# songyb111-gachon/binary-hologram-reinforcement-learning

Measured on AMD Instinct MI355X. Metric: env-steps/sec (1024x1024, 24-plane), higher is better.
Workload: dtype f32

## Files before the change

### binary-hologram-reinforcement-learning_amd/csrc/hbx_passes.hip

```cpp
#include <hip/hip_runtime.h>
#include <stdint.h>

#include "hbx_fft.hpp"
#include "hbx_internal.hpp"
#include "hbx_rowcol.hpp"
#include "hbx_walk_planes.hpp"

namespace hbx {

template <int SK>
__device__ __forceinline__ float2 store_round(float2 v) {
  if constexpr (SK == HBX_PRECISION_BF16_STORE) {
    auto r = [](float x) {
      uint32_t u = __float_as_uint(x);
      u += 0x7fffu + ((u >> 16) & 1u);
      return __uint_as_float(u & 0xffff0000u);
    };
    return make_float2(r(v.x), r(v.y));
  } else if constexpr (SK == HBX_PRECISION_F16_STORE) {
    return make_float2((float)(_Float16)v.x, (float)(_Float16)v.y);
  } else {
    return v;
  }
}

template <int SK>
__device__ __forceinline__ float2 store_round_a(float2 v) {
  if constexpr (SK == HBX_PRECISION_F16_STORE) {
    return make_float2(2.0f * (float)(_Float16)(0.5f * v.x), 2.0f * (float)(_Float16)(0.5f * v.y));
  } else {
    return store_round<SK>(v);
  }
}

template <int R>
constexpr int kRowNT = row_nt(R);

template <int R>
constexpr int kPanel = panel_rows(R);

template <int R>
using LayoutA = PanelLine<R, R * R / 2, pan_a(R)>;
template <int R>
using LayoutB = PanelLine<R, R * R, pan_b(R)>;

template <int R>
struct TileB {
  static constexpr int N = R * R, TL = 256 / R;
  __device__ static constexpr int at(int s, int y) {
    return (y >> 4) * 16 * N + (s / TL) * 16 * TL + (y & 15) * TL + s % TL;
  }
};
template <int R>
constexpr bool kTiledB = R == 32 || R == 16;



template <int R>
constexpr int rowfwd_iters() { return R == 32 ? 4 : (R == 16 ? 2 : 1); }

__device__ __forceinline__ JobDesc first_pass_job(const JobDesc* jobs, const int64_t* actions, int32_t* err,
                                                  int j, bool writer, int64_t hw, int P, int CH) {
  if (!actions) return jobs[j];
  const JobDesc jb = job_of_action(actions[j], j, hw, P, CH);
  if (writer && threadIdx.x == 0) {
    const_cast<JobDesc*>(jobs)[j] = jb;
    if (jb.env < 0 && err) atomicOr(err, 1);
  }
  return jb;
}

template <int R, int NT>
constexpr int rowfwd_scratch() {
  static_assert(R * R * (NT / R) <= (NT / R) * R * (R + 1), "tile must fit in the scratch area");
  return (NT / R) * R * (R + 1);
}

template <int R, int NT, int SK>
__device__ __forceinline__ void rowfwd_emit(pk2 (&v)[R], int t, int grp, int lane_base, int y0, float2* lds,
                                            const float2* tw, float2* __restrict__ base) {
  constexpr int N = R * R;
  constexpr int GPB = NT / R;
  constexpr size_t PLA = plane_a_elems(R);
  fft_group<R, false>(v, t, PaddedScratch<R>{lds + grp * R * (R + 1)}, tw);
  lds_barrier();

  float2* tile = lds;
  const float2 zny = from_pk(v[R / 2]);
#pragma unroll
  for (int k2 = 0; k2 < R / 2; ++k2) {
    const float2 z = from_pk(v[k2]);
    const float2 m = mirror_conj<R>(v, k2, t, lane_base);
    float2 fa = make_float2(z.x + m.x, z.y + m.y);
    float2 fb = make_float2(z.y - m.y, m.x - z.x);
    if (k2 == 0 && t == 0) {
      fa = make_float2(z.x + z.x, zny.x + zny.x);
      fb = make_float2(z.y + z.y, zny.y + zny.y);
    }
    const int kx = t + R * k2;
    tile[tile_pos<R, GPB>(kx, grp)] = fa;
    tile[tile_pos<R, GPB>(N / 2 + kx, grp)] = fb;
  }
  lds_barrier();
  constexpr int CHUNKS = N * GPB / 2;
  static_assert(CHUNKS % NT == 0, "chunking");
#pragma unroll
  for (int i = 0; i < CHUNKS / NT; ++i) {
    const int c = threadIdx.x + NT * i;
    const int r2 = (c % (GPB / 2)) * 2;
    const int line = c / (GPB / 2);
    float2 a, b;
    if constexpr (GPB == 16) {
      const int p0 = tile_pos<R, GPB>(line, r2);
      const float4 ab = *reinterpret_cast<const float4*>(tile + (p0 & ~1));
      const bool sw = (p0 & 1) != 0;
      a = sw ? make_float2(ab.z, ab.w) : make_float2(ab.x, ab.y);
      b = sw ? make_float2(ab.x, ab.y) : make_float2(ab.z, ab.w);
    } else {
      a = tile[tile_pos<R, GPB>(line, r2)];
      b = tile[tile_pos<R, GPB>(line, r2 + 1)];
    }
    a = store_round_a<SK>(a);
    b = store_round_a<SK>(b);
    const int pl = line / (N / 2);
    st_stream4(base + (size_t)pl * PLA + LayoutA<R>::at(line - pl * (N / 2), y0 + r2),
               make_float4(a.x, a.y, b.x, b.y));
  }
}

template <int R, int NT, int SK, int RIT = rowfwd_iters<R>()>
__global__ __launch_bounds__(NT, 512 / NT) void k_rowfwd(const JobDesc* jobs,
                                                   const uint32_t* __restrict__ mask,
                                                   float2* __restrict__ ws_a,
                                                   const float2* __restrict__ tw_glob, int P,
                                                   int CH, float va, float vb, int pair_step,
                                                   const int64_t* __restrict__ actions, int32_t* err,
                                                   const uint8_t* __restrict__ phase) {
  constexpr int N = R * R;
  constexpr int GPB = NT / R;
  constexpr int WPR = N / 32;
  __shared__ float2 tw[N];
  __shared__ __attribute__((aligned(16))) float2 lds[rowfwd_scratch<R, NT>()];

  stage_twiddles<N, NT>(tw, tw_glob);

  const int grp = threadIdx.x / R;
  const int t = threadIdx.x % R;
  const int lane_base = (threadIdx.x & 63) - t;
  constexpr int RB = N / GPB;
  constexpr int RBW = RB / RIT;
  const FirstPassBlock wg = first_pass_block<RBW>(RIT == 1 ? xcd_pair<RB>(blockIdx.x) : (int)blockIdx.x,
                                                  pair_step ? 1 : P / 2);
  const int rbw = wg.rbw, j = wg.j;
  const JobDesc jb = first_pass_job(jobs, actions, err, j, wg.writer, (int64_t)N * N, P, CH);
  if (jb.env < 0 || (phase && phase[j])) return;
  const int q = pair_step ? (jb.flip_plane >> 1) : wg.q;
  const int pa = 2 * q, pb = 2 * q + 1;
  const uint32_t* plane_a = mask + ((size_t)jb.env * CH + jb.group * P + pa) * N * WPR;
  uint32_t wa[WPR], wb[WPR];
  auto load_row = [&](int y) {
    const uint32_t* rowa = plane_a + (size_t)y * WPR;
    const uint32_t* rowb = rowa + (size_t)N * WPR;
    if constexpr (WPR % 4 == 0) {
#pragma unroll
      for (int i = 0; i < WPR / 4; ++i) {
        const uint4 a = reinterpret_cast<const uint4*>(rowa)[i];
        const uint4 b = reinterpret_cast<const uint4*>(rowb)[i];
        wa[4 * i] = a.x; wa[4 * i + 1] = a.y; wa[4 * i + 2] = a.z; wa[4 * i + 3] = a.w;
        wb[4 * i] = b.x; wb[4 * i + 1] = b.y; wb[4 * i + 2] = b.z; wb[4 * i + 3] = b.w;
      }
    } else {
#pragma unroll
      for (int i = 0; i < WPR; ++i) { wa[i] = rowa[i]; wb[i] = rowb[i]; }
    }
  };
  load_row(rbw * RIT * GPB + grp);
  __syncthreads();

  float2* base = ws_a + ((size_t)j * P + pa) * plane_a_elems(R);
  int it = 0;
#pragma unroll 1
  do {
    const int y0 = (rbw * RIT + it) * GPB;
    const int y = y0 + grp;
    if (jb.flip_plane >= 0 && jb.flip_pix / N == y) {
      const int col = jb.flip_pix % N;
      const uint32_t bit = 1u << (col & 31);
#pragma unroll
      for (int i = 0; i < WPR; ++i) {
        if (i == (col >> 5)) {
          if (jb.flip_plane == pa) wa[i] ^= bit;
          if (jb.flip_plane == pb) wb[i] ^= bit;
        }
      }
    }
    pk2 v[R];
    with_field_kind(va, vb, [&](auto fk) {
#pragma unroll
      for (int jj = 0; jj < R; ++jj) {
        const int w = (R * jj) >> 5;
        const int sh = ((R * jj) & 31) + t;
        v[jj] = (pk2){bit_value<fk()>(wa[w], sh, va, vb), bit_value<fk()>(wb[w], sh, va, vb)};
      }
    });
    if constexpr (RIT > 1) {
      load_row(it + 1 < RIT ? y + GPB : y);
      if (it > 0) lds_barrier();
    }
    rowfwd_emit<R, NT, SK>(v, t, grp, lane_base, y0, lds, tw, base);
  } while (RIT > 1 && ++it < RIT);
}

constexpr int kRowfwd32Scr = 8 * 32 * (32 + 1);
static_assert((1024 / 2) * 8 * 2 <= kRowfwd32Scr, "one plane's tile must fit in the FFT tiles");

template <int SK>
__device__ __forceinline__ void rowfwd32_emit(pk2 (&v)[32], int t, int k1, int grp, int y0, float* lds,
                                              const float2* tw, float2* __restrict__ base) {
  constexpr int R = 32, NT = 256, N = R * R, GPB = NT / R;
  constexpr size_t PLA = plane_a_elems(R);
  float2* tile = reinterpret_cast<float2*>(lds);
  fft_group_split_mirror<false>(v, t, k1, lds + grp * R * (R + 1), tw);

  float2 fb[R / 2];
  lds_barrier();
  const float2 zny = from_pk(v[R / 2]);
#pragma unroll
  for (int k2 = 0; k2 < R / 2; ++k2) {
    const float2 z = from_pk(v[k2]);
    const float2 m = mirror_conj_paired(v, k2, t);
    float2 fa = make_float2(z.x + m.x, z.y + m.y);
    fb[k2] = make_float2(z.y - m.y, m.x - z.x);
    if (k2 == 0 && t == 0) {
      fa = make_float2(z.x + z.x, zny.x + zny.x);
      fb[k2] = make_float2(z.y + z.y, zny.y + zny.y);
    }
    tile[tile_pos<R, GPB>(k1 + R * k2, grp)] = fa;
  }
  constexpr int CHUNKS = (N / 2) * GPB / 2;
  static_assert(CHUNKS % NT == 0, "chunking");
#pragma unroll
  for (int pl = 0; pl < 2; ++pl) {
    if (pl == 1) {
      lds_barrier();
#pragma unroll
      for (int k2 = 0; k2 < R / 2; ++k2) tile[tile_pos<R, GPB>(k1 + R * k2, grp)] = fb[k2];
    }
    lds_barrier();
#pragma unroll
    for (int i = 0; i < CHUNKS / NT; ++i) {
      const int c = threadIdx.x + NT * i;
      const int r2 = (c % (GPB / 2)) * 2;
      const int line = c / (GPB / 2);
      const float2 a = store_round_a<SK>(tile[tile_pos<R, GPB>(line, r2)]);
      const float2 b = store_round_a<SK>(tile[tile_pos<R, GPB>(line, r2 + 1)]);
      st_stream4(base + (size_t)pl * PLA + LayoutA<R>::at(line, y0 + r2), make_float4(a.x, a.y, b.x, b.y));
    }
  }
}

template <int SK, int RIT = rowfwd_iters<32>()>
__global__ __launch_bounds__(256, 3) void k_rowfwd32(const JobDesc* jobs,
                                                     const uint32_t* __restrict__ mask,
                                                     float2* __restrict__ ws_a,
                                                     const float2* __restrict__ tw_glob, int P, int CH,
                                                     float va, float vb, int pair_step,
                                                     const int64_t* __restrict__ actions, int32_t* err,
                                                     const uint8_t* __restrict__ phase) {
  constexpr int R = 32, NT = 256, N = R * R;
  constexpr int GPB = NT / R;
  constexpr int WPR = N / 32;
  __shared__ float2 tw[N];
  __shared__ __attribute__((aligned(16))) float lds[kRowfwd32Scr];

  stage_twiddles<N, NT>(tw, tw_glob);

  const int grp = threadIdx.x / R;
  const int t = threadIdx.x % R;
  const int k1 = mirror_k1(t);
  constexpr int RB = N / GPB;
  constexpr int RBW = RB / RIT;
  int bid = RIT == 1 ? xcd_pair<RB>(blockIdx.x) : (int)blockIdx.x;
  const int rbw = bid % RBW;
  bid /= RBW;
  const int npair = pair_step ? 1 : P / 2;
  const int j = bid / npair;
  const JobDesc jb = first_pass_job(jobs, actions, err, j, rbw == 0 && bid % npair == 0, (int64_t)N * N, P, CH);
  if (jb.env < 0 || (phase && phase[j])) return;
  const int q = pair_step ? (jb.flip_plane >> 1) : bid % npair;
  const int pa = 2 * q, pb = 2 * q + 1;
  const uint32_t* plane_a = mask + ((size_t)jb.env * CH + jb.group * P + pa) * N * WPR;
  uint32_t wa, wb;
  auto load_row = [&](int y) {
    wa = plane_a[(size_t)y * WPR + t];
    wb = plane_a[(size_t)(N + y) * WPR + t];
  };
  load_row(rbw * RIT * GPB + grp);
  __syncthreads();

  float2* base = ws_a + ((size_t)j * P + pa) * plane_a_elems(R);
  int it = 0;
#pragma unroll 1
  do {
    const int y0 = (rbw * RIT + it) * GPB;
    const int y = y0 + grp;
    uint32_t ta = group_bit_transpose(wa, t);
    uint32_t tb = group_bit_transpose(wb, t);
    if (jb.flip_plane >= 0 && jb.flip_pix / N == y) {
      const int col = jb.flip_pix % N;
      if (t == (col & 31)) {
        if (jb.flip_plane == pa) ta ^= 1u << (col >> 5);
        if (jb.flip_plane == pb) tb ^= 1u << (col >> 5);
      }
    }
    pk2 v[R];
    with_field_kind(va, vb, [&](auto fk) {
#pragma unroll
      for (int jj = 0; jj < R; ++jj)
        v[jj] = (pk2){bit_value<fk()>(ta, jj, va, vb), bit_value<fk()>(tb, jj, va, vb)};
    });
    if constexpr (RIT > 1) {
      load_row(it + 1 < RIT ? y + GPB : y);
      if (it > 0) lds_barrier();
    }
    rowfwd32_emit<SK>(v, t, k1, grp, y0, lds, tw, base);
  } while (RIT > 1 && ++it < RIT);
}

template <int R, int NT>
__global__ __launch_bounds__(NT, 512 / NT) void k_rowfwd_real(const JobDesc* __restrict__ jobs,
                                                        const float* __restrict__ values,
                                                        float2* __restrict__ ws_a,
                                                        const float2* __restrict__ tw_glob, int P, int CH) {
  constexpr int N = R * R;
  constexpr int GPB = NT / R;
  __shared__ float2 tw[N];
  __shared__ __attribute__((aligned(16))) float2 lds[rowfwd_scratch<R, NT>()];

  stage_twiddles<N, NT>(tw, tw_glob);

  const int grp = threadIdx.x / R;
  const int t = threadIdx.x % R;
  const int lane_base = (threadIdx.x & 63) - t;
  constexpr int RB = N / GPB;
  const FirstPassBlock wg = first_pass_block<RB>(xcd_pair<RB>(blockIdx.x), P / 2);
  const int j = wg.j;
  const JobDesc jb = jobs[j];
  if (jb.env < 0) return;
  const int pa = 2 * wg.q;
  const int y0 = wg.rbw * GPB;
  const int y = y0 + grp;
  pk2 v[R];
  real_load_row<R>(v, values + (((size_t)jb.env * CH + jb.group * P + pa) * N + y) * N, (size_t)N * N, t);
  __syncthreads();

  float2* base = ws_a + ((size_t)j * P + pa) * plane_a_elems(R);
  rowfwd_emit<R, NT, HBX_PRECISION_F32>(v, t, grp, lane_base, y0, lds, tw, base);
}

__global__ __launch_bounds__(256, 3) void k_rowfwd32_real(const JobDesc* __restrict__ jobs,
                                                          const float* __restrict__ values,
                                                          float2* __restrict__ ws_a,
                                                          const float2* __restrict__ tw_glob, int P, int CH) {
  constexpr int R = 32, NT = 256, N = R * R;
  constexpr int GPB = NT / R;
  __shared__ float2 tw[N];
  __shared__ __attribute__((aligned(16))) float lds[kRowfwd32Scr];

  stage_twiddles<N, NT>(tw, tw_glob);

  const int grp = threadIdx.x / R;
  const int t = threadIdx.x % R;
  const int k1 = mirror_k1(t);
  constexpr int RB = N / GPB;
  const FirstPassBlock wg = first_pass_block<RB>(xcd_pair<RB>(blockIdx.x), P / 2);
  const int j = wg.j;
  const JobDesc jb = jobs[j];
  if (jb.env < 0) return;
  const int pa = 2 * wg.q;
  const int y0 = wg.rbw * GPB;
  const int y = y0 + grp;
  pk2 v[R];
  real_load_row<R>(v, values + (((size_t)jb.env * CH + jb.group * P + pa) * N + y) * N, (size_t)N * N, t);
  __syncthreads();

  float2* base = ws_a + ((size_t)j * P + pa) * plane_a_elems(R);
  rowfwd32_emit<HBX_PRECISION_F32>(v, t, k1, grp, y0, lds, tw, base);
}

template <int R, int NT, bool WT = false>
__global__ __launch_bounds__(NT, 512 / NT) void k_rowfwd_cplx(const JobDesc* __restrict__ jobs,
                                                        const float2* __restrict__ values,
                                                        float2* __restrict__ ws_a,
                                                        const float2* __restrict__ tw_glob, int P, int CH,
                                                        const float* __restrict__ weight, float scale) {
  constexpr int N = R * R;
  constexpr int GPB = NT / R;
  __shared__ float2 tw[N];
  __shared__ __attribute__((aligned(16))) float2 lds[rowfwd_scratch<R, NT>()];

  stage_twiddles<N, NT>(tw, tw_glob);

  const int grp = threadIdx.x / R;
  const int t = threadIdx.x % R;
  const int lane_base = (threadIdx.x & 63) - t;
  constexpr int RB = N / GPB;
  const FirstPassBlock wg = first_pass_block<RB>(xcd_pair<RB>(blockIdx.x), P / 2);
  const int j = wg.j;
  const JobDesc jb = jobs[j];
  if (jb.env < 0) return;
  const int y0 = wg.rbw * GPB;
  const int y = y0 + grp;
  pk2 v[R];
  const float2* row = values + (((size_t)jb.env * (CH / 2) + jb.group * (P / 2) + wg.q) * N + y) * N;
  if constexpr (WT)
    complex_load_row_weighted<R>(v, row, weight + (((size_t)jb.env * (CH / P) + jb.group) * N + y) * N, scale, t);
  else
    complex_load_row<R>(v, row, t);
  __syncthreads();

  float2* base = ws_a + ((size_t)j * P + 2 * wg.q) * plane_a_elems(R);
  rowfwd_emit<R, NT, HBX_PRECISION_F32>(v, t, grp, lane_base, y0, lds, tw, base);
}

template <bool WT = false>
__global__ __launch_bounds__(256, 3) void k_rowfwd32_cplx(const JobDesc* __restrict__ jobs,
                                                          const float2* __restrict__ values,
                                                          float2* __restrict__ ws_a,
                                                          const float2* __restrict__ tw_glob, int P, int CH,
                                                          const float* __restrict__ weight, float scale) {
  constexpr int R = 32, NT = 256, N = R * R;
  constexpr int GPB = NT / R;
  __shared__ float2 tw[N];
  __shared__ __attribute__((aligned(16))) float lds[kRowfwd32Scr];

  stage_twiddles<N, NT>(tw, tw_glob);

  const int grp = threadIdx.x / R;
  const int t = threadIdx.x % R;
  const int k1 = mirror_k1(t);
  constexpr int RB = N / GPB;
  const FirstPassBlock wg = first_pass_block<RB>(xcd_pair<RB>(blockIdx.x), P / 2);
  const int j = wg.j;
  const JobDesc jb = jobs[j];
  if (jb.env < 0) return;
  const int y0 = wg.rbw * GPB;
  const int y = y0 + grp;
  pk2 v[R];
  const float2* row = values + (((size_t)jb.env * (CH / 2) + jb.group * (P / 2) + wg.q) * N + y) * N;
  if constexpr (WT)
    complex_load_row_weighted<R>(v, row, weight + (((size_t)jb.env * (CH / P) + jb.group) * N + y) * N, scale, t);
  else
    complex_load_row<R>(v, row, t);
  __syncthreads();

  float2* base = ws_a + ((size_t)j * P + 2 * wg.q) * plane_a_elems(R);
  rowfwd32_emit<HBX_PRECISION_F32>(v, t, k1, grp, y0, lds, tw, base);
}

template <int R>
__host__ __device__ constexpr int col2_iters() { return R == 32 ? 4 : (R == 16 ? 2 : 1); }

template <int R, int SK>
__device__ __forceinline__ void col2_stage_write(const float2 (&v)[R], float sy, float2* scratch, int grp, int t) {
  constexpr int PQ = R >= 32 ? 1 : 32 / R;
  float2* reg = col2_region<R>(scratch, grp);
  float2* base[PQ];
#pragma unroll
  for (int q = 0; q < PQ; ++q) base[q] = reg + col2_pos<R>(grp >> 1, t + R * q);
#pragma unroll
  for (int q = 0; q < PQ; ++q) {
#pragma unroll
    for (int k2 = q; k2 < R; k2 += PQ) base[q][R * (k2 - q)] = store_round<SK>(make_float2(v[k2].x, sy * v[k2].y));
  }
}

template <int R, int SK, int ITER = col2_iters<R>()>
__global__ __launch_bounds__(256, 2) void k_col2(const JobDesc* __restrict__ jobs,
                                                 const float2* __restrict__ ws_a,
                                                 float2* __restrict__ ws_b,
                                                 const float2* __restrict__ htab,
                                                 const float2* __restrict__ tw_glob, int P,
                                                 int pair_step, const uint8_t* __restrict__ phase) {
  constexpr int N = R * R;
  constexpr int GPB = 256 / R;
  constexpr int LB = (N / 2) / (GPB * ITER);
  static_assert((N / 2) % (GPB * ITER) == 0, "line blocking");
  __shared__ float2 tw[N];
  constexpr int RS = kTiledB<R> ? col2_region_stride<R>() : R * (R + 1);
  __shared__ float2 scratch[GPB * RS];

  for (int i = threadIdx.x; i < N; i += 256) tw[i] = tw_glob[i];

  const int grp = threadIdx.x / R;
  const int t = threadIdx.x % R;
  const int lane_base = (threadIdx.x & 63) - t;
  int bid = blockIdx.x;
  const int lb = bid % LB;
  bid /= LB;
  const int np = pair_step ? 2 : P;
  const int j = bid / np;
  const JobDesc jb = jobs[j];
  if (jb.env < 0 || (phase && phase[j])) return;
  const int p = pair_step ? (jb.flip_plane & ~1) + bid % 2 : bid % np;
  using PA = LayoutA<R>;
  using PB = LayoutB<R>;
  const __amdgpu_buffer_rsrc_t ra = plane_rsrc(ws_a + ((size_t)j * P + p) * plane_a_elems(R), plane_a_elems(R) * 8);
  const __amdgpu_buffer_rsrc_t rb = plane_rsrc(ws_b + ((size_t)j * P + p) * plane_b_elems(R), plane_b_elems(R) * 8);
  const __amdgpu_buffer_rsrc_t rh = plane_rsrc(htab + (size_t)jb.group * (N / 2 + 1) * N, (N / 2 + 1) * N * 8);
  const PaddedScratch<R> sc{scratch + grp * RS};
  constexpr int KSTEP = LB * GPB;
  const int kx0 = lb * GPB + grp;

  float2 v[R];
  {
    const int vo = PA::voff(t, kx0);
#pragma unroll
    for (int jj = 0; jj < R; ++jj) v[jj] = buf_ld2s(ra, vo, PA::joff(jj));
  }
  lds_barrier();

#pragma unroll 1
  for (int it = 0; it < ITER; ++it) {
    const int kx = kx0 + it * KSTEP;
    const bool dc = (kx == 0);
    const int vh = (kx * N + t) * 8;
    constexpr int HP = kTiledB<R> ? R / 2 + 1 : 0;
    float2 hb[R];
    if constexpr (kTiledB<R>) {
      fft_group_s1<R, false, true>(v, t, tw);
      if (!dc) {
#pragma unroll
        for (int i = 0; i < HP; ++i) hb[i] = buf_ld2(rh, vh, i * R * 8);
      }
      if (it > 0) lds_barrier();
      fft_group_s2<R, false, true>(v, t, sc);
    } else {
      fft_group<R, false, true>(v, t, sc, tw);
    }
    float2 w[R];
    if (!dc) {
      if constexpr (kTiledB<R>) {
        float2* hs = scratch + grp * RS;
        wave_sync();
#pragma unroll
        for (int i = 0; i <= R / 2; ++i) hs[i * R + t] = hb[i];
        wave_sync();
        const float2* hm = hs + (t == 0 ? R : 0) + ((R - t) & (R - 1));
#pragma unroll
        for (int i = R / 2 + 1; i < R; ++i) hb[i] = hm[(R - 1 - i) * R];
        wave_sync();
      } else {
#pragma unroll
        for (int i = 0; i < R; ++i) hb[i] = buf_ld2(rh, vh, i * R * 8);
      }
#pragma unroll
      for (int i = 0; i < R; ++i) {
        w[i] = cmulc(v[i], hb[i]);
        v[i] = cmul(v[i], hb[i]);
      }
    } else {
      const int vn = ((N / 2) * N + t) * 8;
#pragma unroll
      for (int k2 = 0; k2 < R; ++k2) w[k2] = mirror_conj<R>(v, k2, t, lane_base);
#pragma unroll
      for (int k2 = 0; k2 < R; ++k2) {
        const float2 z = v[k2], mm = w[k2];
        v[k2] = cmul(make_float2(0.5f * (z.x + mm.x), 0.5f * (z.y + mm.y)), buf_ld2(rh, vh, k2 * R * 8));
        w[k2] = cmul(make_float2(0.5f * (z.y - mm.y), -0.5f * (z.x - mm.x)), buf_ld2(rh, vn, k2 * R * 8));
      }
    }
    fft_group<R, true, true>(v, t, sc, tw);
    const float sy = dc ? 1.0f : -1.0f;
    if constexpr (kTiledB<R>) {
      const int kxb = kx - grp;
      col2_stage_write<R, SK>(v, 1.0f, scratch, grp, t);
      lds_barrier();
      col2_stage_store<R>(scratch, rb, kxb / GPB);
      if (it + 1 < ITER) {
        const int vo = PA::voff(t, kx + KSTEP);
#pragma unroll
        for (int jj = 0; jj < R; ++jj) v[jj] = buf_ld2s(ra, vo, PA::joff(jj));
      }
      fft_group_s1<R, true, true>(w, t, tw);
      lds_barrier();
      fft_group_s2<R, true, true>(w, t, sc);
      col2_stage_write<R, SK>(w, sy, scratch, grp, t);
      lds_barrier();
      col2_stage_store<R>(scratch, rb, (N / 2 + kxb) / GPB);
    } else {
      {
        const int vo = PB::voff(t, kx);
#pragma unroll
        for (int k2 = 0; k2 < R; ++k2) buf_st2s(store_round<SK>(v[k2]), rb, vo, PB::joff(k2));
      }
      if (it + 1 < ITER) {
        const int vo = PA::voff(t, kx + KSTEP);
#pragma unroll
        for (int jj = 0; jj < R; ++jj) v[jj] = buf_ld2s(ra, vo, PA::joff(jj));
      }
      fft_group<R, true, true>(w, t, sc, tw);
      {
        const int vo = PB::voff(t, dc ? N / 2 : N - kx);
#pragma unroll
        for (int k2 = 0; k2 < R; ++k2)
          buf_st2s(store_round<SK>(make_float2(w[k2].x, sy * w[k2].y)), rb, vo, PB::joff(k2));
      }
    }
  }
}

template <int R, int GPB, bool SC1 = false, bool TPRE = false>
__device__ __forceinline__ void rowinv_epilogue(float (&acc)[R], int P, int G, const JobDesc& jb, int j, int y,
                                                int rb, int grp, int t, const float* __restrict__ target,
                                                size_t tmask, float* __restrict__ inten_out, int inten_by_env,
                                                double* __restrict__ partial, double (&red)[GPB][3],
                                                const int32_t* __restrict__ rc_pending = nullptr,
                                                float* __restrict__ rc_cache = nullptr,
                                                const float* tpre = nullptr) {
  constexpr int N = R * R;
  constexpr int RB = N / GPB;
  const float invp = 1.0f / (float)P;
  const float* trow = target + ((((size_t)jb.env * G + jb.group) * N + y) * N & tmask);
  double sxy = 0.0, sxx = 0.0, syy = 0.0;
#pragma unroll
  for (int k = 0; k < R; ++k) {
    const float I = acc[k] * invp;
    const float T = TPRE ? tpre[k] : trow[t + R * k];
    sxy = fma((double)I, (double)T, sxy);
    sxx = fma((double)I, (double)I, sxx);
    syy = fma((double)T, (double)T, syy);
    acc[k] = I;
  }
  if (inten_out) {
    const size_t slot = inten_by_env ? (size_t)jb.env * G + jb.group : (size_t)j;
    float* orow = inten_out + (slot * N + y) * N;
    if (rc_pending) {
      const int p = rc_pending[jb.env];
      if (p != 0) {
        const int gp = (p > 0 ? p : -p) - 1;
        const size_t grow = (((size_t)jb.env * G + gp) * N + y) * N;
        if (p > 0) {
#pragma unroll
          for (int k = 0; k < R; ++k) rc_cache[grow + t + R * k] = inten_out[grow + t + R * k];
        } else if (gp != jb.group) {
#pragma unroll
          for (int k = 0; k < R; ++k) inten_out[grow + t + R * k] = rc_cache[grow + t + R * k];
        }
      }
    }
    if (inten_by_env) {
#pragma unroll
      for (int k = 0; k < R; ++k) __builtin_nontemporal_store(acc[k], orow + t + R * k);
    } else {
#pragma unroll
      for (int k = 0; k < R; ++k) orow[t + R * k] = acc[k];
    }
  }
#pragma unroll
  for (int off = R / 2; off >= 1; off >>= 1) {
    sxy += __shfl_xor(sxy, off, 64);
    sxx += __shfl_xor(sxx, off, 64);
    syy += __shfl_xor(syy, off, 64);
  }
  if (t == 0) { red[grp][0] = sxy; red[grp][1] = sxx; red[grp][2] = syy; }
  __syncthreads();
  if (threadIdx.x == 0) {
    double a = 0.0, b = 0.0, cc = 0.0;
    for (int g = 0; g < GPB; ++g) { a += red[g][0]; b += red[g][1]; cc += red[g][2]; }
    double* o = partial + ((size_t)j * RB + rb) * 3;
    if constexpr (SC1) {
      const __amdgpu_buffer_rsrc_t ro = walk_planes_rsrc(o, 24);
      __builtin_amdgcn_raw_buffer_store_b64(__builtin_bit_cast(u32x2, a), ro, 0, 0, kSc1Bit);
      __builtin_amdgcn_raw_buffer_store_b64(__builtin_bit_cast(u32x2, b), ro, 8, 0, kSc1Bit);
      __builtin_amdgcn_raw_buffer_store_b64(__builtin_bit_cast(u32x2, cc), ro, 16, 0, kSc1Bit);
    } else {
      o[0] = a; o[1] = b; o[2] = cc;
    }
  }
}

template <int R>
struct RowinvLanes {
  static constexpr int N = R * R, TL = 256 / R;
  static constexpr int JS = 16 * R * 8;
  int lo, hiB, vmid;
  __device__ __forceinline__ RowinvLanes(int y, int t) {
    const int yb = (y >> 4) * 16 * N + (y & 15) * TL;
    const int m = t / TL, u = t % TL;
    lo = (yb + m * 16 * TL + u) * 8;
    hiB = (yb + (u ? (3 * N / (2 * TL) - m - 1) * 16 * TL + TL - u : (3 * N / (2 * TL) - m) * 16 * TL) -
           16 * R * (R - 1)) * 8;
    vmid = t == 0 ? lo + JS * (R / 2) : hiB + JS * (R / 2 - 1);
  }
  __device__ __forceinline__ float2 load(__amdgpu_buffer_rsrc_t rs, int po, int jj) const {
    const int vo = jj < R / 2 ? lo : (jj == R / 2 ? vmid : hiB);
    const int so = po + (jj < R / 2 ? JS * jj : (jj == R / 2 ? 0 : JS * (R - 1 - jj)));
    return buf_ld2s(rs, vo, so);
  }
};

template <int R, bool WALK = false, bool LEAN = false>
__global__ __launch_bounds__(256, 2) void k_rowinv_d(const JobDesc* __restrict__ jobs,
                                                     const float2* __restrict__ ws_b,
                                                     const float* __restrict__ target,
                                                     const float2* __restrict__ tw_glob, int P, int G,
                                                     double* __restrict__ partial, float* __restrict__ inten_out,
                                                     float2* __restrict__ field_out, size_t tmask, int inten_by_env,
                                                     int plane_mode, float* __restrict__ plane_pool,
                                                     const int32_t* __restrict__ plane_slot, int plane_spares,
                                                     int spare_base, const int32_t* __restrict__ rc_pending,
                                                     float* __restrict__ rc_cache, WalkPlanesArgs wk) {
  constexpr int N = R * R, GPB = 256 / R, RB = N / GPB;
  static_assert(!WALK || walk_planes_lds_bytes(RB) <= GPB * R * (R + 1) * 8, "the decision's LDS fits the scratch");
  __shared__ float2 tw[N];
  __shared__ float2 scratch[GPB * R * (R + 1)];
  __shared__ double red[GPB][3];
  for (int i = threadIdx.x; i < N; i += 256) tw[i] = tw_glob[i];

  const int grp = threadIdx.x / R;
  const int t = threadIdx.x % R;
  const int bid = xcd_pair<RB>(blockIdx.x);
  const int rb = bid % RB;
  const int j = bid / RB;
  const JobDesc jb = jobs[j];
  if constexpr (WALK) {
    if (wk.phase && wk.phase[j] == 2) {
      walk_planes_arrive(wk, reinterpret_cast<char*>(scratch));
      return;
    }
  }
  if (jb.env < 0) {
    if (threadIdx.x == 0) {
      double* o = partial + ((size_t)j * RB + rb) * 3;
      if constexpr (WALK) {
        const __amdgpu_buffer_rsrc_t ro = walk_planes_rsrc(o, 24);
        for (int i = 0; i < 3; ++i) __builtin_amdgcn_raw_buffer_store_b64(u32x2{0u, 0u}, ro, 8 * i, 0, kSc1Bit);
      } else {
        o[0] = 0.0; o[1] = 0.0; o[2] = 0.0;
      }
    }
    if constexpr (WALK) walk_planes_arrive(wk, reinterpret_cast<char*>(scratch));
    return;
  }
  if constexpr (LEAN) {
    plane_mode = kPlanesOff;
    field_out = nullptr;
    rc_pending = nullptr;
    rc_cache = nullptr;
  }
  const int y = rb * GPB + grp;
  constexpr int PLB = N * N;
  const __amdgpu_buffer_rsrc_t rs = plane_rsrc(ws_b + (size_t)j * P * PLB, (unsigned)((size_t)P * PLB * 8));
  const RowinvLanes<R> ln(y, t);
  auto load_plane = [&](pk2 (&v)[R], int p) {
    const int po = p * PLB * 8;
#pragma unroll
    for (int jj = 0; jj < R; ++jj) v[jj] = to_pk(ln.load(rs, po, jj));
  };
  float acc[R];
#pragma unroll
  for (int k = 0; k < R; ++k) acc[k] = 0.0f;
  const PaddedScratch<R> sc{scratch + grp * R * (R + 1)};
  const int CH = G * P;
  const int CHS = CH + 2 * (plane_spares > 1 ? plane_spares : 1);
  const int spare = CH + 2 * (plane_spares > 1 ? spare_base + j : 0);
  const int32_t* slots = plane_slot ? plane_slot + (size_t)jb.env * CHS : nullptr;
  auto pool_row = [&](int slot) { return plane_pool + (((size_t)jb.env * CHS + slot) * N + y) * N; };
  auto finish_plane = [&](pk2 (&v)[R], int p) {
    fft_group<R, true>(v, t, sc, tw);
    float f[R];
#pragma unroll
    for (int k = 0; k < R; ++k) {
      f[k] = fmaf(v[k].x, v[k].x, v[k].y * v[k].y);
      acc[k] += f[k];
    }
    if (field_out) {
      float2* frow = field_out + (((size_t)jb.env * G * P + jb.group * P + p) * N + y) * N;
#pragma unroll
      for (int k = 0; k < R; ++k) frow[t + R * k] = from_pk(v[k]);
    }
    if (plane_mode != kPlanesOff) {
      float* orow = pool_row(slots[plane_mode == kPlanesFill ? jb.group * P + p : spare + (p & 1)]);
#pragma unroll
      for (int k = 0; k < R; ++k) __builtin_nontemporal_store(f[k], orow + t + R * k);
    }
  };
  auto add_cached = [&](int q) {
    const float* crow = pool_row(slots[jb.group * P + q]);
    float c[R];
#pragma unroll
    for (int k = 0; k < R; ++k) c[k] = __builtin_nontemporal_load(crow + t + R * k);
#pragma unroll
    for (int k = 0; k < R; ++k) acc[k] += c[k];
  };
  pk2 va[R];
  if (plane_mode == kPlanesStep) {
    const int pa = jb.flip_plane & ~1;
    load_plane(va, pa);
    __syncthreads();
#pragma unroll 1
    for (int q = 0; q < pa; ++q) add_cached(q);
    finish_plane(va, pa);
    load_plane(va, pa + 1);
    finish_plane(va, pa + 1);
#pragma unroll 1
    for (int q = pa + 2; q < P; ++q) add_cached(q);
    rowinv_epilogue<R, GPB, WALK>(acc, P, G, jb, j, y, rb, grp, t, target, tmask, inten_out, inten_by_env, partial,
                                  red, rc_pending, rc_cache);
    if constexpr (WALK) {
      __syncthreads();
      walk_planes_arrive(wk, reinterpret_cast<char*>(scratch));
    }
    return;
  }
  load_plane(va, 0);
  __syncthreads();
  if constexpr (R == 16) {
    pk2 vb[R];
#pragma unroll 1
    for (int p = 0; p < P; p += 2) {
      load_plane(vb, p + 1);
      finish_plane(va, p);
      load_plane(va, p + 2 < P ? p + 2 : p + 1);
      finish_plane(vb, p + 1);
    }
  } else if constexpr (LEAN) {
#pragma unroll 1
    for (int p = 0; p < P - 1; ++p) {
      finish_plane(va, p);
      load_plane(va, p + 1);
    }
    const float* trow = target + ((((size_t)jb.env * G + jb.group) * N + y) * N & tmask);
    float tv[R];
#pragma unroll
    for (int k = 0; k < R; ++k) tv[k] = trow[t + R * k];
    finish_plane(va, P - 1);
    rowinv_epilogue<R, GPB, false, true>(acc, P, G, jb, j, y, rb, grp, t, target, tmask, inten_out, inten_by_env,
                                         partial, red, rc_pending, rc_cache, tv);
    return;
  } else {
#pragma unroll 1
    for (int p = 0; p < P; ++p) {
      finish_plane(va, p);
      load_plane(va, p + 1 < P ? p + 1 : p);
    }
  }
  rowinv_epilogue<R, GPB>(acc, P, G, jb, j, y, rb, grp, t, target, tmask, inten_out, inten_by_env, partial, red,
                           rc_pending, rc_cache);
}

template <int R, int NT>
__global__ __launch_bounds__(NT, 512 / NT) void k_rowinv(const JobDesc* __restrict__ jobs,
                                                   const float2* __restrict__ ws_b,
                                                   const float* __restrict__ target,
                                                   const float2* __restrict__ tw_glob, int P,
                                                   int G, double* __restrict__ partial,
                                                   float* __restrict__ inten_out,
                                                   float2* __restrict__ field_out,
                                                   size_t tmask, int inten_by_env) {
  constexpr int N = R * R;
  constexpr int GPB = NT / R;
  constexpr int RB = N / GPB;
  constexpr int CH16 = N * GPB / 2;
  constexpr int PER = CH16 / NT;
  static_assert(CH16 % NT == 0, "chunking");
  constexpr int SCR = GPB * R * (R + 1);
  __shared__ float2 tw[N];
  __shared__ __attribute__((aligned(16))) float2 tile[SCR > N * GPB ? SCR : N * GPB];
  __shared__ double red[GPB][3];

  for (int i = threadIdx.x; i < N; i += NT) tw[i] = tw_glob[i];

  const int grp = threadIdx.x / R;
  const int t = threadIdx.x % R;
  const int bid = xcd_pair<RB>(blockIdx.x);
  const int rb = bid % RB;
  const int j = bid / RB;
  const JobDesc jb = jobs[j];
  if (jb.env < 0) {
    if (threadIdx.x == 0) {
      double* o = partial + ((size_t)j * RB + rb) * 3;
      o[0] = 0.0; o[1] = 0.0; o[2] = 0.0;
    }
    return;
  }
  const int y0 = rb * GPB;
  const int y = y0 + grp;
  constexpr size_t PLB = plane_b_elems(R);
  const float2* jbase = ws_b + (size_t)j * P * PLB;

  float4 pre[PER];
#pragma unroll
  for (int i = 0; i < PER; ++i) {
    const int c = threadIdx.x + NT * i;
    const int line = c / (GPB / 2), r2 = (c % (GPB / 2)) * 2;
    pre[i] = ld_stream4(jbase + LayoutB<R>::at(line, y0 + r2));
  }
  float acc[R];
#pragma unroll
  for (int k = 0; k < R; ++k) acc[k] = 0.0f;

#pragma unroll 1
  for (int p = 0; p < P; ++p) {
    lds_barrier();
#pragma unroll
    for (int i = 0; i < PER; ++i) {
      const int c = threadIdx.x + NT * i;
      const int line = c / (GPB / 2), r2 = (c % (GPB / 2)) * 2;
      tile[tile_pos<R, GPB>(line, r2)] = make_float2(pre[i].x, pre[i].y);
      tile[tile_pos<R, GPB>(line, r2 + 1)] = make_float2(pre[i].z, pre[i].w);
    }
    if (p + 1 < P) {
      const float2* nb = jbase + (size_t)(p + 1) * PLB;
#pragma unroll
      for (int i = 0; i < PER; ++i) {
        const int c = threadIdx.x + NT * i;
        const int line = c / (GPB / 2), r2 = (c % (GPB / 2)) * 2;
        pre[i] = ld_stream4(nb + LayoutB<R>::at(line, y0 + r2));
      }
    }
    lds_barrier();
    pk2 v[R];
#pragma unroll
    for (int jj = 0; jj < R; ++jj) v[jj] = to_pk(tile[tile_pos<R, GPB>(t + R * jj, grp)]);
    lds_barrier();
    fft_group<R, true>(v, t, PaddedScratch<R>{tile + grp * R * (R + 1)}, tw);
#pragma unroll
    for (int k = 0; k < R; ++k) acc[k] += fmaf(v[k].x, v[k].x, v[k].y * v[k].y);
    if (field_out) {
      float2* frow = field_out + (((size_t)jb.env * G * P + jb.group * P + p) * N + y) * N;
#pragma unroll
      for (int k = 0; k < R; ++k) frow[t + R * k] = from_pk(v[k]);
    }
  }

  rowinv_epilogue<R, GPB>(acc, P, G, jb, j, y, rb, grp, t, target, tmask, inten_out, inten_by_env, partial, red);
}

template <int R>
__global__ __launch_bounds__(256, 2) void k_rowinv_d_cplx(const JobDesc* __restrict__ jobs,
                                                          const float2* __restrict__ ws_b,
                                                          const float2* __restrict__ tw_glob, int P, int G,
                                                          float2* __restrict__ field_out,
                                                          float* __restrict__ real_out) {
  constexpr int N = R * R, GPB = 256 / R, RB = N / GPB;
  __shared__ float2 tw[N];
  __shared__ float2 scratch[GPB * R * (R + 1)];
  for (int i = threadIdx.x; i < N; i += 256) tw[i] = tw_glob[i];

  const int grp = threadIdx.x / R;
  const int t = threadIdx.x % R;
  const int bid = xcd_pair<RB>(blockIdx.x);
  const int rb = bid % RB;
  const int j = bid / RB;
  const JobDesc jb = jobs[j];
  if (jb.env < 0) return;
  const int y = rb * GPB + grp;
  const int Q = P / 2;
  constexpr int PLB = N * N;
  const __amdgpu_buffer_rsrc_t rs = plane_rsrc(ws_b + (size_t)j * P * PLB, (unsigned)((size_t)P * PLB * 8));
  const RowinvLanes<R> ln(y, t);
  auto load_pair = [&](pk2 (&v)[R], int q) {
    const int po = 2 * q * PLB * 8;
#pragma unroll
    for (int jj = 0; jj < R; ++jj) v[jj] = to_pk(ln.load(rs, po, jj));
#pragma unroll
    for (int h = 0; h < 2; ++h) {
      float2 w[R / 2];
#pragma unroll
      for (int jj = 0; jj < R / 2; ++jj) w[jj] = ln.load(rs, po + PLB * 8, h * (R / 2) + jj);
#pragma unroll
      for (int jj = 0; jj < R / 2; ++jj) {
        v[h * (R / 2) + jj].x -= w[jj].y;
        v[h * (R / 2) + jj].y += w[jj].x;
      }
    }
  };
  const PaddedScratch<R> sc{scratch + grp * R * (R + 1)};
  const size_t row0 = (((size_t)jb.env * G + jb.group) * Q * N + y) * N + t;
  auto finish_plane = [&](pk2 (&v)[R], int q) {
    fft_group<R, true>(v, t, sc, tw);
    const size_t row = row0 + (size_t)q * N * N;
    if (field_out) {
#pragma unroll
      for (int k = 0; k < R; ++k) field_out[row + R * k] = from_pk(v[k]);
    }
    if (real_out) {
#pragma unroll
      for (int k = 0; k < R; ++k) real_out[row + R * k] = v[k].x;
    }
  };
  pk2 va[R];
  load_pair(va, 0);
  __syncthreads();
  if constexpr (R == 16) {
    pk2 vb[R];
#pragma unroll 1
    for (int q = 0; q < Q; q += 2) {
      if (q + 1 < Q) load_pair(vb, q + 1);
      finish_plane(va, q);
      if (q + 1 < Q) {
        if (q + 2 < Q) load_pair(va, q + 2);
        finish_plane(vb, q + 1);
      }
    }
  } else {
#pragma unroll 1
    for (int q = 0; q < Q; ++q) {
      finish_plane(va, q);
      if (q + 1 < Q) load_pair(va, q + 1);
    }
  }
}

template <int R, int NT>
__global__ __launch_bounds__(NT, 512 / NT) void k_rowinv_cplx(const JobDesc* __restrict__ jobs,
                                                        const float2* __restrict__ ws_b,
                                                        const float2* __restrict__ tw_glob, int P, int G,
                                                        float2* __restrict__ field_out,
                                                        float* __restrict__ real_out) {
  constexpr int N = R * R;
  constexpr int GPB = NT / R;
  constexpr int RB = N / GPB;
  constexpr int CH16 = N * GPB / 2;
  constexpr int PER = CH16 / NT;
  static_assert(CH16 % NT == 0, "chunking");
  constexpr int SCR = GPB * R * (R + 1);
  __shared__ float2 tw[N];
  __shared__ __attribute__((aligned(16))) float2 tile[SCR > N * GPB ? SCR : N * GPB];

  for (int i = threadIdx.x; i < N; i += NT) tw[i] = tw_glob[i];

  const int grp = threadIdx.x / R;
  const int t = threadIdx.x % R;
  const int bid = xcd_pair<RB>(blockIdx.x);
  const int rb = bid % RB;
  const int j = bid / RB;
  const JobDesc jb = jobs[j];
  if (jb.env < 0) return;
  const int y0 = rb * GPB;
  const int y = y0 + grp;
  const int Q = P / 2;
  constexpr size_t PLB = plane_b_elems(R);
  const float2* jbase = ws_b + (size_t)j * P * PLB;

  float4 pa[PER], pb[PER];
  auto load_pair = [&](int q) {
    const float2* a = jbase + (size_t)(2 * q) * PLB;
#pragma unroll
    for (int i = 0; i < PER; ++i) {
      const int c = threadIdx.x + NT * i;
      const int line = c / (GPB / 2), r2 = (c % (GPB / 2)) * 2;
      pa[i] = ld_stream4(a + LayoutB<R>::at(line, y0 + r2));
      pb[i] = ld_stream4(a + PLB + LayoutB<R>::at(line, y0 + r2));
    }
  };
  load_pair(0);
  const size_t row0 = (((size_t)jb.env * G + jb.group) * Q * N + y) * N + t;

#pragma unroll 1
  for (int q = 0; q < Q; ++q) {
    lds_barrier();
#pragma unroll
    for (int i = 0; i < PER; ++i) {
      const int c = threadIdx.x + NT * i;
      const int line = c / (GPB / 2), r2 = (c % (GPB / 2)) * 2;
      tile[tile_pos<R, GPB>(line, r2)] = make_float2(pa[i].x - pb[i].y, pa[i].y + pb[i].x);
      tile[tile_pos<R, GPB>(line, r2 + 1)] = make_float2(pa[i].z - pb[i].w, pa[i].w + pb[i].z);
    }
    if (q + 1 < Q) load_pair(q + 1);
    lds_barrier();
    pk2 v[R];
#pragma unroll
    for (int jj = 0; jj < R; ++jj) v[jj] = to_pk(tile[tile_pos<R, GPB>(t + R * jj, grp)]);
    lds_barrier();
    fft_group<R, true>(v, t, PaddedScratch<R>{tile + grp * R * (R + 1)}, tw);
    const size_t row = row0 + (size_t)q * N * N;
    if (field_out) {
#pragma unroll
      for (int k = 0; k < R; ++k) field_out[row + R * k] = from_pk(v[k]);
    }
    if (real_out) {
#pragma unroll
      for (int k = 0; k < R; ++k) real_out[row + R * k] = v[k].x;
    }
  }
}

template <int R, bool INV>
__global__ __launch_bounds__(256, 2) void k_fft_rt(const float2* __restrict__ in,
                                                   float2* __restrict__ out,
                                                   const float2* __restrict__ tw_glob) {
  constexpr int N = R * R;
  constexpr int GPB = 256 / R;
  constexpr int SCR = GPB * R * (R + 1);
  static_assert(N * GPB <= SCR, "tile must fit in the scratch area");
  constexpr int RB = N / GPB;
  __shared__ float2 tw[N];
  __shared__ __attribute__((aligned(16))) float2 lds[SCR];
  for (int i = threadIdx.x; i < N; i += 256) tw[i] = tw_glob[i];
  const int grp = threadIdx.x / R;
  const int t = threadIdx.x % R;
  int bid = xcd_pair<RB>(blockIdx.x);
  const int rb = bid % RB;
  const int plane = bid / RB;
  const int y0 = rb * GPB;
  const float2* row = in + ((size_t)plane * N + y0 + grp) * N + t;
  float2 v[R];
#pragma unroll
  for (int j = 0; j < R; ++j) v[j] = row[R * j];
  __syncthreads();
  fft_group<R, INV>(v, t, PaddedScratch<R>{lds + grp * R * (R + 1)}, tw);
  lds_barrier();
#pragma unroll
  for (int k2 = 0; k2 < R; ++k2) lds[tile_pos<R>(t + R * k2, grp)] = v[k2];
  lds_barrier();
  float2* base = out + (size_t)plane * N * N;
  constexpr int CHUNKS = N * GPB / 2;
#pragma unroll
  for (int i = 0; i < CHUNKS / 256; ++i) {
    const int c = threadIdx.x + 256 * i;
    const int r2 = (c % (GPB / 2)) * 2;
    const int line = c / (GPB / 2);
    const float2 a = lds[tile_pos<R>(line, r2)];
    const float2 b = lds[tile_pos<R>(line, r2 + 1)];
    *reinterpret_cast<float4*>(base + (size_t)line * N + y0 + r2) = make_float4(a.x, a.y, b.x, b.y);
  }
}

template <int R>
static hipError_t launch_fft2d(const PlanDev& pd, float2* a, float2* b, int n_planes, bool inverse,
                               hipStream_t st) {
  constexpr int N = R * R;
  const unsigned blocks = (unsigned)n_planes * (N / (256 / R));
  for (int pass = 0; pass < 2; ++pass) {
    const float2* src = pass == 0 ? a : b;
    float2* dst = pass == 0 ? b : a;
    if (inverse)
      hipLaunchKernelGGL((k_fft_rt<R, true>), dim3(blocks), dim3(256), 0, st, src, dst, pd.tw);
    else
      hipLaunchKernelGGL((k_fft_rt<R, false>), dim3(blocks), dim3(256), 0, st, src, dst, pd.tw);
  }
  return hipGetLastError();
}

template <bool INV>
__global__ __launch_bounds__(256, 2) void k_fft_rt896(const float2* __restrict__ in,
                                                      float2* __restrict__ out,
                                                      const float2* __restrict__ tw_glob) {
  constexpr int N = 896, R = 32, GPB = 8, RB = N / GPB;
  constexpr int SCR = GPB * R * (R + 1);
  static_assert(N * GPB <= SCR, "tile must fit in the scratch area");
  __shared__ float2 tw[N];
  __shared__ __attribute__((aligned(16))) float2 lds[SCR];
  for (int i = threadIdx.x; i < N; i += 256) tw[i] = tw_glob[i];
  const int grp = threadIdx.x / R;
  const int t = threadIdx.x % R;
  int bid = xcd_pair<RB>(blockIdx.x);
  const int rb = bid % RB;
  const int plane = bid / RB;
  const int y0 = rb * GPB;
  const float2* row = in + ((size_t)plane * N + y0 + grp) * N + t;
  float2 v[32];
#pragma unroll
  for (int j = 0; j < 28; ++j) v[j] = row[R * j];
  __syncthreads();
  fft896_ns<INV>(v, t, PaddedScratch<R>{lds + grp * R * (R + 1)}, tw);
  lds_barrier();
  if (t < 28) {
#pragma unroll
    for (int k2 = 0; k2 < 32; ++k2) lds[tile_pos<R, GPB>(t + 28 * k2, grp)] = v[k2];
  }
  lds_barrier();
  float2* base = out + (size_t)plane * N * N;
  constexpr int CHUNKS = N * GPB / 2;
  static_assert(CHUNKS % 256 == 0, "chunking");
#pragma unroll
  for (int i = 0; i < CHUNKS / 256; ++i) {
    const int c = threadIdx.x + 256 * i;
    const int r2 = (c % (GPB / 2)) * 2;
    const int line = c / (GPB / 2);
    const float2 a = lds[tile_pos<R, GPB>(line, r2)];
    const float2 b = lds[tile_pos<R, GPB>(line, r2 + 1)];
    *reinterpret_cast<float4*>(base + (size_t)line * N + y0 + r2) = make_float4(a.x, a.y, b.x, b.y);
  }
}

hipError_t run_fft2d(const PlanDev& pd, float2* a, float2* b, int n_planes, bool inverse,
                     hipStream_t st) {
  if (n_planes <= 0) return hipSuccess;
  if (pd.R == 0) {
    const unsigned blocks = (unsigned)n_planes * (896 / 8);
    for (int pass = 0; pass < 2; ++pass) {
      const float2* src = pass == 0 ? a : b;
      float2* dst = pass == 0 ? b : a;
      if (inverse) hipLaunchKernelGGL((k_fft_rt896<true>), dim3(blocks), dim3(256), 0, st, src, dst, pd.tw);
      else hipLaunchKernelGGL((k_fft_rt896<false>), dim3(blocks), dim3(256), 0, st, src, dst, pd.tw);
    }
    return hipGetLastError();
  }
  switch (pd.R) {
    case 32: return launch_fft2d<32>(pd, a, b, n_planes, inverse, st);
    case 16: return launch_fft2d<16>(pd, a, b, n_planes, inverse, st);
    case 8: return launch_fft2d<8>(pd, a, b, n_planes, inverse, st);
    default: return hipErrorInvalidValue;
  }
}

__global__ void k_reduce_partials(const double* __restrict__ partial, int n_jobs, int RB,
                                  double* __restrict__ job_stats);

template <int R, int SK>
static hipError_t launch_passes(const PlanDev& pd, const JobDesc* jobs, int n_jobs,
                                const uint32_t* mask, const float* target, float* inten_out,
                                float2* field_out, hipStream_t st) {
  constexpr int N = R * R;
  constexpr int GPB = 256 / R;
  const int P = pd.P;
  const int CH = pd.G * pd.P;
  PassTimer* tm = pd.timer;
  const int pair = pd.plane_mode == kPlanesStep ? 1 : 0;
  if (pd.plane_mode != kPlanesOff && (!kTiledB<R> || !pd.plane_pool || !pd.plane_slot)) return hipErrorInvalidValue;
  constexpr unsigned kSmallBlocks = 2048;
  const unsigned rf_blocks = (unsigned)n_jobs * (pair ? 1 : P / 2) * (N / (kRowNT<R> / R)) / rowfwd_iters<R>();
  const unsigned col_blocks = (unsigned)n_jobs * (pair ? 2 : P) * ((N / 2) / (GPB * col2_iters<R>()));
  const bool small = kTiledB<R> && rf_blocks < kSmallBlocks && col_blocks < kSmallBlocks;
  if (pd.complex_values && (SK != HBX_PRECISION_F32 || pd.plane_mode != kPlanesOff || pd.actions || pd.walk_phase ||
                            pd.real_values || (!pd.complex_field && !pd.real_part)))
    return hipErrorInvalidValue;
  if (pd.complex_weight && !pd.complex_values) return hipErrorInvalidValue;
  {
    if (tm) tm->begin(0, st);
    if (pd.complex_values) {
      const unsigned blocks = (unsigned)n_jobs * (P / 2) * (N / (kRowNT<R> / R));
      const float* cw = pd.complex_weight;
      const float cs = pd.complex_scale;
      if constexpr (R == 32) {
        if (cw)
          hipLaunchKernelGGL(k_rowfwd32_cplx<true>, dim3(blocks), dim3(256), 0, st, jobs, pd.complex_values, pd.ws_a,
                             pd.tw, P, CH, cw, cs);
        else
          hipLaunchKernelGGL(k_rowfwd32_cplx<false>, dim3(blocks), dim3(256), 0, st, jobs, pd.complex_values, pd.ws_a,
                             pd.tw, P, CH, cw, cs);
      } else {
        if (cw)
          hipLaunchKernelGGL((k_rowfwd_cplx<R, kRowNT<R>, true>), dim3(blocks), dim3(kRowNT<R>), 0, st, jobs,
                             pd.complex_values, pd.ws_a, pd.tw, P, CH, cw, cs);
        else
          hipLaunchKernelGGL((k_rowfwd_cplx<R, kRowNT<R>, false>), dim3(blocks), dim3(kRowNT<R>), 0, st, jobs,
                             pd.complex_values, pd.ws_a, pd.tw, P, CH, cw, cs);
      }
    } else if (pd.real_values) {
      if (SK != HBX_PRECISION_F32 || pair || pd.actions || pd.walk_phase) return hipErrorInvalidValue;
      const unsigned blocks = (unsigned)n_jobs * (P / 2) * (N / (kRowNT<R> / R));
      if constexpr (R == 32)
        hipLaunchKernelGGL(k_rowfwd32_real, dim3(blocks), dim3(256), 0, st, jobs, pd.real_values, pd.ws_a, pd.tw, P,
                           CH);
      else
        hipLaunchKernelGGL((k_rowfwd_real<R, kRowNT<R>>), dim3(blocks), dim3(kRowNT<R>), 0, st, jobs,
                           pd.real_values, pd.ws_a, pd.tw, P, CH);
    } else if constexpr (R == 32) {
      if (small)
        hipLaunchKernelGGL((k_rowfwd32<SK, 1>), dim3(rf_blocks * rowfwd_iters<R>()), dim3(256), 0, st, jobs, mask,
                           pd.ws_a, pd.tw, P, CH, pd.va, pd.vb, pair, pd.actions, pd.act_err, pd.walk_phase);
      else
        hipLaunchKernelGGL((k_rowfwd32<SK>), dim3(rf_blocks), dim3(256), 0, st, jobs, mask, pd.ws_a, pd.tw, P, CH,
                           pd.va, pd.vb, pair, pd.actions, pd.act_err, pd.walk_phase);
    } else if constexpr (kTiledB<R>) {
      if (small)
        hipLaunchKernelGGL((k_rowfwd<R, kRowNT<R>, SK, 1>), dim3(rf_blocks * rowfwd_iters<R>()), dim3(kRowNT<R>), 0,
                           st, jobs, mask, pd.ws_a, pd.tw, P, CH, pd.va, pd.vb, pair, pd.actions, pd.act_err, pd.walk_phase);
      else
        hipLaunchKernelGGL((k_rowfwd<R, kRowNT<R>, SK>), dim3(rf_blocks), dim3(kRowNT<R>), 0, st, jobs, mask,
                           pd.ws_a, pd.tw, P, CH, pd.va, pd.vb, pair, pd.actions, pd.act_err, pd.walk_phase);
    } else {
      hipLaunchKernelGGL((k_rowfwd<R, kRowNT<R>, SK>), dim3(rf_blocks), dim3(kRowNT<R>), 0, st, jobs, mask, pd.ws_a,
                         pd.tw, P, CH, pd.va, pd.vb, pair, pd.actions, pd.act_err, pd.walk_phase);
    }
    if (tm) tm->end(0, n_jobs, st);
  }
  {
    if (tm) tm->begin(1, st);
    if constexpr (kTiledB<R>) {
      if (small)
        hipLaunchKernelGGL((k_col2<R, SK, 1>), dim3(col_blocks * col2_iters<R>()), dim3(256), 0, st, jobs, pd.ws_a,
                           pd.ws_b, pd.htab, pd.tw, P, pair, pd.walk_phase);
      else
        hipLaunchKernelGGL((k_col2<R, SK>), dim3(col_blocks), dim3(256), 0, st, jobs, pd.ws_a, pd.ws_b, pd.htab,
                           pd.tw, P, pair, pd.walk_phase);
    } else {
      hipLaunchKernelGGL((k_col2<R, SK>), dim3(col_blocks), dim3(256), 0, st, jobs, pd.ws_a, pd.ws_b, pd.htab,
                         pd.tw, P, pair, pd.walk_phase);
    }
    if (tm) tm->end(1, n_jobs, st);
  }
  {
    const unsigned blocks = (unsigned)n_jobs * (N / (kRowNT<R> / R));
    if (tm) tm->begin(2, st);
    if (pd.complex_values) {
      if constexpr (kTiledB<R>)
        hipLaunchKernelGGL((k_rowinv_d_cplx<R>), dim3(blocks), dim3(256), 0, st, jobs, pd.ws_b, pd.tw, P, pd.G,
                           pd.complex_field, pd.real_part);
      else
        hipLaunchKernelGGL((k_rowinv_cplx<R, kRowNT<R>>), dim3(blocks), dim3(kRowNT<R>), 0, st, jobs, pd.ws_b,
                           pd.tw, P, pd.G, pd.complex_field, pd.real_part);
      if (tm) tm->end(2, n_jobs, st);
      return hipGetLastError();
    }
    if constexpr (kTiledB<R>) {
      if (pd.walk_planes) {
        if (pd.plane_mode != kPlanesStep) return hipErrorInvalidValue;
        hipLaunchKernelGGL((k_rowinv_d<R, true>), dim3(blocks), dim3(256), 0, st, jobs, pd.ws_b,
                           target ? target : pd.zero_row, pd.tw, P, pd.G, pd.partial, inten_out, field_out,
                           target ? ~(size_t)0 : (size_t)0, pd.inten_by_env, pd.plane_mode, pd.plane_pool,
                           pd.plane_slot, pd.plane_spares, pd.spare_base, pd.rc_pending, pd.rc_cache,
                           *pd.walk_planes);
      } else if (pd.plane_mode == kPlanesOff && !field_out && !pd.rc_pending) {
        hipLaunchKernelGGL((k_rowinv_d<R, false, true>), dim3(blocks), dim3(256), 0, st, jobs, pd.ws_b,
                           target ? target : pd.zero_row, pd.tw, P, pd.G, pd.partial, inten_out, field_out,
                           target ? ~(size_t)0 : (size_t)0, pd.inten_by_env, pd.plane_mode, pd.plane_pool,
                           pd.plane_slot, pd.plane_spares, pd.spare_base, pd.rc_pending, pd.rc_cache,
                           WalkPlanesArgs{});
      } else {
        hipLaunchKernelGGL((k_rowinv_d<R>), dim3(blocks), dim3(256), 0, st, jobs, pd.ws_b,
                           target ? target : pd.zero_row, pd.tw, P, pd.G, pd.partial, inten_out, field_out,
                           target ? ~(size_t)0 : (size_t)0, pd.inten_by_env, pd.plane_mode, pd.plane_pool,
                           pd.plane_slot, pd.plane_spares, pd.spare_base, pd.rc_pending, pd.rc_cache,
                           WalkPlanesArgs{});
      }
    }
    else
      hipLaunchKernelGGL((k_rowinv<R, kRowNT<R>>), dim3(blocks), dim3(kRowNT<R>), 0, st, jobs, pd.ws_b,
                         target ? target : pd.zero_row, pd.tw, P, pd.G, pd.partial, inten_out,
                         field_out, target ? ~(size_t)0 : (size_t)0, pd.inten_by_env);
    if (tm) tm->end(2, n_jobs, st);
  }
  if (!pd.skip_reduce)
    hipLaunchKernelGGL(k_reduce_partials, dim3(n_jobs), dim3(64), 0, st, pd.partial,
                       n_jobs, N / (kRowNT<R> / R), pd.job_stats);
  return hipGetLastError();
}

hipError_t run_jobs(const PlanDev& pd, const JobDesc* jobs, int n_jobs, const uint32_t* mask,
                    const float* target, float* inten_out, float2* field_out, hipStream_t st) {
  if (pd.R == 0) return run_jobs_896(pd, jobs, n_jobs, mask, target, inten_out, field_out, st);
  switch (pd.R * 4 + pd.store_kind) {
#define HBX_PASSES_CASE(R_, SK_) \
    case R_ * 4 + SK_: return launch_passes<R_, SK_>(pd, jobs, n_jobs, mask, target, inten_out, field_out, st);
    HBX_PASSES_CASE(32, HBX_PRECISION_F32)
    HBX_PASSES_CASE(32, HBX_PRECISION_BF16_STORE)
    HBX_PASSES_CASE(32, HBX_PRECISION_F16_STORE)
    HBX_PASSES_CASE(16, HBX_PRECISION_F32)
    HBX_PASSES_CASE(16, HBX_PRECISION_BF16_STORE)
    HBX_PASSES_CASE(16, HBX_PRECISION_F16_STORE)
    HBX_PASSES_CASE(8, HBX_PRECISION_F32)
    HBX_PASSES_CASE(8, HBX_PRECISION_BF16_STORE)
    HBX_PASSES_CASE(8, HBX_PRECISION_F16_STORE)
#undef HBX_PASSES_CASE
    default: return hipErrorInvalidValue;
  }
}

}
```

Before: 25830.

## Gather second FFT stage through LDS and store 128-bit lines directly for R=32

For the R=32 column pass, the second FFT stage is replaced: after the first stage, each group writes its values to LDS in a permuted column layout, and threads gather across groups to run a scalar DFT. Results are then stored straight to global memory as 128-bit buffer stores, with DPP lane swaps pairing adjacent outputs. This removes the separate staged LDS write/read transpose before the global store and changes the memory access pattern. The cost is new LDS bank behaviour, cross-lane shuffles and a per-lane sign computation for the DC term, and the correctness of the new output layout is hard to verify.

Result: no change. 25790, median of 2 (-0.2%).

```diff
diff --git a/binary-hologram-reinforcement-learning_amd/csrc/hbx_passes.hip b/binary-hologram-reinforcement-learning_amd/csrc/hbx_passes.hip
--- a/binary-hologram-reinforcement-learning_amd/csrc/hbx_passes.hip
+++ b/binary-hologram-reinforcement-learning_amd/csrc/hbx_passes.hip
@@ -475,6 +475,47 @@
   }
 }
 
+template <int R>
+constexpr bool kGatherB = R == 32;
+template <int R>
+__host__ __device__ constexpr int col2_gather_stride() { return R * (R + 1) + 2; }
+__host__ __device__ constexpr int col2_gcol(int k1) { return (k1 & 1) | ((k1 >> 2) << 1) | (((k1 >> 1) & 1) << 4); }
+
+template <int R, int RS>
+__device__ __forceinline__ void col2_gather_dft(float2 (&v)[R], float2* scratch, int grp, int t) {
+  constexpr int TL = 256 / R;
+  float2* wr = scratch + grp * RS + t * (R + 1);
+#pragma unroll
+  for (int k1 = 0; k1 < R; ++k1) wr[col2_gcol(k1)] = v[k1];
+  lds_barrier();
+  const int lane = threadIdx.x & 63, s = lane % TL;
+  const int k1 = (64 / TL) * (threadIdx.x >> 6) + lane / TL;
+  const float2* rd = scratch + s * RS + col2_gcol(k1);
+#pragma unroll
+  for (int tt = 0; tt < R; ++tt) v[tt] = rd[tt * (R + 1)];
+  dft_reg_scalar<R, true>(v);
+}
+template <int R, int SK>
+__device__ __forceinline__ void col2_gather_store(const float2 (&v)[R], float sy, __amdgpu_buffer_rsrc_t rb, int st) {
+  static_assert(R == 32, "two waves per 16-row band");
+  constexpr int N = R * R, TL = 256 / R;
+  const int w = threadIdx.x >> 6, lane = threadIdx.x & 63;
+  const bool odd = lane & 1;
+  const int vo = ((w >> 1) * 16 * N + st * 16 * TL + (w & 1) * 64 + (lane & ~1)) * 8 + (odd ? 2 * 16 * N * 8 : 0);
+#pragma unroll
+  for (int j = 0; j < R / 2; ++j) {
+    const float2 a = store_round<SK>(make_float2(v[2 * j].x, sy * v[2 * j].y));
+    const float2 b = store_round<SK>(make_float2(v[2 * j + 1].x, sy * v[2 * j + 1].y));
+    const float2 snd = odd ? a : b;
+    float2 rcv;
+    rcv.x = __uint_as_float((uint32_t)__builtin_amdgcn_mov_dpp((int)__float_as_uint(snd.x), 0xB1, 0xf, 0xf, false));
+    rcv.y = __uint_as_float((uint32_t)__builtin_amdgcn_mov_dpp((int)__float_as_uint(snd.y), 0xB1, 0xf, 0xf, false));
+    const float2 lo = odd ? rcv : a, hi = odd ? b : rcv;
+    const u32x4 o = {__float_as_uint(lo.x), __float_as_uint(lo.y), __float_as_uint(hi.x), __float_as_uint(hi.y)};
+    __builtin_amdgcn_raw_buffer_store_b128(o, rb, vo + j * 4 * 16 * N * 8, 0, kBufNT);
+  }
+}
+
 template <int R, int SK, int ITER = col2_iters<R>()>
 __global__ __launch_bounds__(256, 2) void k_col2(const JobDesc* __restrict__ jobs,
                                                  const float2* __restrict__ ws_a,
@@ -487,7 +528,8 @@
   constexpr int LB = (N / 2) / (GPB * ITER);
   static_assert((N / 2) % (GPB * ITER) == 0, "line blocking");
   __shared__ float2 tw[N];
-  constexpr int RS = kTiledB<R> ? col2_region_stride<R>() : R * (R + 1);
+  constexpr int RS = kGatherB<R> ? col2_gather_stride<R>()
+                                 : (kTiledB<R> ? col2_region_stride<R>() : R * (R + 1));
   __shared__ float2 scratch[GPB * RS];
 
   for (int i = threadIdx.x; i < N; i += 256) tw[i] = tw_glob[i];
@@ -570,8 +612,25 @@
         w[k2] = cmul(make_float2(0.5f * (z.y - mm.y), -0.5f * (z.x - mm.x)), buf_ld2(rh, vn, k2 * R * 8));
       }
     }
+    const float sy = dc ? 1.0f : -1.0f;
+    if constexpr (kGatherB<R>) {
+      const int kxb = kx - grp;
+      fft_group_s1<R, true, true>(v, t, tw);
+      wave_sync();
+      col2_gather_dft<R, RS>(v, scratch, grp, t);
+      col2_gather_store<R, SK>(v, 1.0f, rb, kxb / GPB);
+      if (it + 1 < ITER) {
+        const int vo = PA::voff(t, kx + KSTEP);
+#pragma unroll
+        for (int jj = 0; jj < R; ++jj) v[jj] = buf_ld2s(ra, vo, PA::joff(jj));
+      }
+      fft_group_s1<R, true, true>(w, t, tw);
+      lds_barrier();
+      col2_gather_dft<R, RS>(w, scratch, grp, t);
+      col2_gather_store<R, SK>(w, kxb + (int)(threadIdx.x & 63) % GPB == 0 ? 1.0f : -1.0f, rb, (N / 2 + kxb) / GPB);
+      continue;
+    }
     fft_group<R, true, true>(v, t, sc, tw);
-    const float sy = dc ? 1.0f : -1.0f;
     if constexpr (kTiledB<R>) {
       const int kxb = kx - grp;
       col2_stage_write<R, SK>(v, 1.0f, scratch, grp, t);
```
